# facebookresearch/NasRec

Measured on AMD Instinct MI355X. Metric: supernet samples/sec at batch 256 (Criteo-shape), 1/2/4/8 MI355X, higher is better.
Workload: dtype f32

## Files before the change

### nasrec_amd/csrc/worklist_body.h

```cpp
#pragma once
#include "attention_tok.h"
#include "gemm_rt.h"
#include "final_bodies.h"
#include "interact_bodies.h"
#include "dedup_bodies.h"

#define WL_LDS_BIG_FLOATS 9888
#define WL_LDS_FLOATS 7840
static_assert(MHA_TOK_BWD_LDS_FLOATS <= WL_LDS_BIG_FLOATS && MHA_TOK_FWD_LDS_FLOATS <= WL_LDS_FLOATS, "Transformer bodies fit the worklist launches");

#define WL_TK 64
#ifndef WL_AUX_RING2
#define WL_AUX_RING2 0
#endif
enum { WL_TOKS = 0, WL_T32x32 = 1, WL_T64x16 = 2, WL_T16x64 = 3 };

extern __shared__ __attribute__((aligned(16))) float wl_lds[];

template <typename T>
__device__ __forceinline__ const T& wl_ref(unsigned long long addr) {
  const unsigned lo = __builtin_amdgcn_readfirstlane((unsigned)addr), hi = __builtin_amdgcn_readfirstlane((unsigned)(addr >> 32));
  return *(const T*)(const __attribute__((address_space(4))) T*)(((unsigned long long)hi << 32) | lo);
}

template <bool KCA, bool KCB, int TBM, int TBN, bool AUX>
__device__ __forceinline__ void wl_gemm_cfg(unsigned long long blob, int vb_, int gx_, int gy_) {
  constexpr int RING = (AUX && !WL_AUX_RING2) ? 1 : 2;
  const nasrec_gemm_desc_t& g = wl_ref<nasrec_gemm_desc_t>(blob);
  const int vb = __builtin_amdgcn_readfirstlane(vb_), gx = __builtin_amdgcn_readfirstlane(gx_), gy = __builtin_amdgcn_readfirstlane(gy_);
  const int nprob = g.zmode ? g.nseg : 1;
  int Mmax = 0, Nmax = 0;
  for (int q = 0; q < nprob; ++q) {
    Mmax = max(Mmax, g.seg[q].M);
    Nmax = max(Nmax, g.seg[q].N);
  }
  const int bx = vb % gx, by = (vb / gx) % gy, bz = vb / (gx * gy);
  gemm_tile_rt<KCA, KCB, 256, WL_TK, TBM, TBN, AUX, RING>(g, Mmax, Nmax, bx, by, bz, wl_lds);
}

template <bool KCA, bool KCB, bool AUX>
__device__ __forceinline__ void wl_gemm_tile(int tile, unsigned long long off, int vb, int gx, int gy) {
  switch (tile) {
    case WL_T32x32: wl_gemm_cfg<KCA, KCB, 32, 32, AUX>(off, vb, gx, gy); break;
    case WL_T64x16: wl_gemm_cfg<KCA, KCB, 64, 16, AUX>(off, vb, gx, gy); break;
    default: wl_gemm_cfg<KCA, KCB, 16, 64, AUX>(off, vb, gx, gy); break;
  }
}

template <bool AUX>
__device__ __forceinline__ void wl_gemm_bind(int bind, int tile, unsigned long long off, int vb, int gx, int gy) {
  if (bind == 0) wl_gemm_tile<true, true, AUX>(tile, off, vb, gx, gy);
  else if (bind == 1) wl_gemm_tile<true, false, AUX>(tile, off, vb, gx, gy);
  else wl_gemm_tile<false, false, AUX>(tile, off, vb, gx, gy);
}

__device__ __forceinline__ void wl_warm_blob(unsigned long long addr, int bytes) {
  int sink, off;
  asm volatile(
      "s_mov_b32 %1, 0\n"
      "1:\n"
      "s_load_dword %0, %2, %1\n"
      "s_add_u32 %1, %1, 64\n"
      "s_cmp_lt_u32 %1, %3\n"
      "s_cbranch_scc1 1b\n"
      "s_waitcnt lgkmcnt(0)"
      : "=&s"(sink), "=&s"(off)
      : "s"(addr), "s"(bytes)
      : "scc", "memory");
}

#define WL_TOK_DEPTH 4
__device__ __forceinline__ void wl_token_fwd(unsigned long long blob, int vb_, int MT_) {
  const nasrec_gemm_desc_t& g = wl_ref<nasrec_gemm_desc_t>(blob);
  const int vb = __builtin_amdgcn_readfirstlane(vb_), MT = __builtin_amdgcn_readfirstlane(MT_);
  const int lane = threadIdx.x & 63, wave = __builtin_amdgcn_readfirstlane(threadIdx.x >> 6);
  const int e = lane & 15, fg = lane >> 4;
  wl_warm_blob(blob, (int)offsetof(nasrec_gemm_desc_t, seg) + g.nseg * (int)sizeof(nasrec_gemm_seg_t));
  const nasrec_gemm_seg_t& s0 = g.seg[0];
  const int M = s0.M, B = s0.N >> 4;
  const int unit = vb * 4 + wave;
  const int b = unit / MT, mt = unit - b * MT;
  if (b >= B) return;
  const int row = min(mt * 16 + e, M - 1);
  f32x4 acc = {0.f, 0.f, 0.f, 0.f};
  f32x4 fa[WL_TOK_DEPTH];
  float fb[WL_TOK_DEPTH][4];
  int lim[WL_TOK_DEPTH];
  int fq = 0, fk = 0;
  auto fetch = [&](int slot) {
    const bool in = fq < g.nseg;
    const nasrec_gemm_seg_t& sg = g.seg[in ? fq : 0];
    const bool live = in && sg.A != nullptr && sg.K > 0;
    const int K = live ? sg.K : 0, kk = fk + 4 * fg;
    lim[slot] = K - fk;
    const __amdgpu_buffer_rsrc_t ra =
        __builtin_amdgcn_make_buffer_rsrc(const_cast<float*>(sg.A), 0, live ? (int)(4 * ((long)(M - 1) * sg.lda + K)) : 0, 0x00020000);
    const __amdgpu_buffer_rsrc_t rb =
        __builtin_amdgcn_make_buffer_rsrc(const_cast<float*>(sg.B + (long)b * sg.ldb), 0, live ? 64 * K : 0, 0x00020000);
    fa[slot] = __builtin_bit_cast(f32x4, __builtin_amdgcn_raw_buffer_load_b128(ra, 4 * (row * sg.lda + kk), 0, 0));
#pragma unroll
    for (int j = 0; j < 4; ++j) fb[slot][j] = __builtin_bit_cast(float, __builtin_amdgcn_raw_buffer_load_b32(rb, 64 * (kk + j) + 4 * e, 0, 0));
    fk += 16;
    const bool next = fk >= K;
    fq = next ? fq + 1 : fq;
    fk = next ? 0 : fk;
  };
  auto multiply = [&](int slot) {
    const int l = lim[slot];
    if (l <= 0) return;
    f32x4 a = fa[slot];
    if (l < 16) {
#pragma unroll
      for (int j = 0; j < 4; ++j) a[j] = 4 * fg + j < l ? a[j] : 0.f;
    }
#pragma unroll
    for (int j = 0; j < 4; ++j) acc = __builtin_amdgcn_mfma_f32_16x16x4f32(a[j], fb[slot][j], acc, 0, 0, 0);
  };
  int steps = 0;
  for (int q = 0; q < g.nseg; ++q) steps += (g.seg[q].A && g.seg[q].K > 0) ? (g.seg[q].K + 15) >> 4 : 1;
#pragma unroll
  for (int r = 0; r < WL_TOK_DEPTH; ++r) fetch(r);
  for (int t = 0; t < steps; t += WL_TOK_DEPTH) {
#pragma unroll
    for (int r = 0; r < WL_TOK_DEPTH; ++r) {
      multiply(r);
      fetch(r);
    }
  }
  {
    const float v4[4] = {acc[0], acc[1], acc[2], acc[3]};
    if (mt * 16 + 4 * fg < M) epilogue_store_col4<NASREC_CM_TOKJ>(g, s0, mt * 16 + 4 * fg, b * 16 + e, M, v4);
  }
}

#define WL_DENSE_STEPS 8
__device__ __forceinline__ void wl_dense_small(unsigned long long blob, int vb_, int NT_, int MTNB_) {
  const nasrec_gemm_desc_t& g = wl_ref<nasrec_gemm_desc_t>(blob);
  const int vb = __builtin_amdgcn_readfirstlane(vb_), NT = __builtin_amdgcn_readfirstlane(NT_);
  const int MT = __builtin_amdgcn_readfirstlane(MTNB_) & 0xffff, NB = __builtin_amdgcn_readfirstlane(MTNB_) >> 16;
  const int lane = threadIdx.x & 63, wave = __builtin_amdgcn_readfirstlane(threadIdx.x >> 6);
  const int e = lane & 15, fg = lane >> 4;
  wl_warm_blob(blob, (int)offsetof(nasrec_gemm_desc_t, seg) + g.nseg * (int)sizeof(nasrec_gemm_seg_t));
  const nasrec_gemm_seg_t& s0 = g.seg[0];
  const int M = s0.M, N = s0.N;
  const int unit = vb * 4 + wave;
  if (unit >= MT * NT) return;
  const int mt = unit / NT, nt = unit - mt * NT;
  const int row = min(mt * 16 + e, M - 1), col = min(nt * 16 + e, N - 1);
  f32x4 fa[WL_DENSE_STEPS], fb[WL_DENSE_STEPS];
  int lim[WL_DENSE_STEPS];
  int fq = 0, fk = 0;
  f32x4 acc = {0.f, 0.f, 0.f, 0.f};
  for (int batch = 0; batch < NB; ++batch) {
#pragma unroll
  for (int slot = 0; slot < WL_DENSE_STEPS; ++slot) {
    const bool in = fq < g.nseg;
    const nasrec_gemm_seg_t& sg = g.seg[in ? fq : 0];
    const bool live = in && sg.A != nullptr && sg.K > 0;
    const int K = live ? sg.K : 0, kk = fk + 4 * fg;
    lim[slot] = K - fk;
    const __amdgpu_buffer_rsrc_t ra =
        __builtin_amdgcn_make_buffer_rsrc(const_cast<float*>(sg.A), 0, live ? (int)(4 * ((long)(M - 1) * sg.lda + K)) : 0, 0x00020000);
    const __amdgpu_buffer_rsrc_t rb =
        __builtin_amdgcn_make_buffer_rsrc(const_cast<float*>(sg.B), 0, live ? (int)(4 * ((long)(N - 1) * sg.ldb + K)) : 0, 0x00020000);
    fa[slot] = __builtin_bit_cast(f32x4, __builtin_amdgcn_raw_buffer_load_b128(ra, 4 * (row * sg.lda + kk), 0, 0));
    fb[slot] = __builtin_bit_cast(f32x4, __builtin_amdgcn_raw_buffer_load_b128(rb, 4 * (col * sg.ldb + kk), 0, 0));
    fk += 16;
    const bool next = fk >= K;
    fq = next ? fq + 1 : fq;
    fk = next ? 0 : fk;
  }
  if (batch == 0 && g.bias) {
    const float warm = g.bias[g.bias_on_rows ? row : col];
    asm volatile("" ::"v"(warm));
  }
#pragma unroll
  for (int slot = 0; slot < WL_DENSE_STEPS; ++slot) {
    const int l = lim[slot];
    if (l > 0) {
      f32x4 a = fa[slot], b = fb[slot];
      if (l < 16) {
#pragma unroll
        for (int j = 0; j < 4; ++j) {
          const bool in = 4 * fg + j < l;
          a[j] = in ? a[j] : 0.f;
          b[j] = in ? b[j] : 0.f;
        }
      }
#pragma unroll
      for (int j = 0; j < 4; ++j) acc = __builtin_amdgcn_mfma_f32_16x16x4f32(a[j], b[j], acc, 0, 0, 0);
    }
  }
  }
  {
    const float v4[4] = {acc[0], acc[1], acc[2], acc[3]};
    if (mt * 16 + 4 * fg < M && nt * 16 + e < N) epilogue_store_col4<NASREC_CM_PLAIN>(g, s0, mt * 16 + 4 * fg, nt * 16 + e, M, v4);
  }
}

__device__ __forceinline__ void wl_dense_small_dx(unsigned long long blob, int vb_, int TU_) {
  const nasrec_gemm_desc_t& g = wl_ref<nasrec_gemm_desc_t>(blob);
  const int vb = __builtin_amdgcn_readfirstlane(vb_), TU = __builtin_amdgcn_readfirstlane(TU_);
  const int lane = threadIdx.x & 63, wave = __builtin_amdgcn_readfirstlane(threadIdx.x >> 6);
  const int e = lane & 15, fg = lane >> 4;
  wl_warm_blob(blob, (int)offsetof(nasrec_gemm_desc_t, seg) + g.nseg * (int)sizeof(nasrec_gemm_seg_t));
  int t = vb * 4 + wave, q = 0;
  if (t >= TU) return;
  while (q < g.nseg - 1 && t >= ((g.seg[q].M + 15) >> 4) * ((g.seg[q].N + 15) >> 4)) t -= ((g.seg[q].M + 15) >> 4) * ((g.seg[q].N + 15) >> 4), ++q;
  const nasrec_gemm_seg_t& sg = g.seg[q];
  const int M = sg.M, N = sg.N, K = sg.K, NT = (N + 15) >> 4;
  const int mt = t / NT, nt = t - mt * NT;
  if (!sg.A || K <= 0) {
    if (!sg.accumulate) {
#pragma unroll
      for (int r = 0; r < 4; ++r) {
        const int i = mt * 16 + 4 * fg + r, j = nt * 16 + e;
        if (i < M && j < N) epilogue_store<NASREC_CM_PLAIN>(g, sg, i, j, 0.f);
      }
    }
    return;
  }
  const int row = min(mt * 16 + e, M - 1), col = min(nt * 16 + e, N - 1);
  const __amdgpu_buffer_rsrc_t ra = __builtin_amdgcn_make_buffer_rsrc(const_cast<float*>(sg.A), 0, (int)(4 * ((long)(M - 1) * sg.lda + K)), 0x00020000);
  const float* wp = sg.B + col;
  f32x4 fa[WL_DENSE_STEPS];
  float fb[WL_DENSE_STEPS][4];
#pragma unroll
  for (int s = 0; s < WL_DENSE_STEPS; ++s) {
    fa[s] = __builtin_bit_cast(f32x4, __builtin_amdgcn_raw_buffer_load_b128(ra, 4 * (row * sg.lda + 16 * s + 4 * fg), 0, 0));
#pragma unroll
    for (int j = 0; j < 4; ++j) fb[s][j] = wp[(long)min(16 * s + 4 * fg + j, K - 1) * sg.ldb];
  }
  if (sg.Aaux) {
    const __amdgpu_buffer_rsrc_t rx = __builtin_amdgcn_make_buffer_rsrc(const_cast<float*>(sg.Aaux), 0, (int)(4 * ((long)(M - 1) * sg.lda + K)), 0x00020000);
    f32x4 fx[WL_DENSE_STEPS];
#pragma unroll
    for (int s = 0; s < WL_DENSE_STEPS; ++s) fx[s] = __builtin_bit_cast(f32x4, __builtin_amdgcn_raw_buffer_load_b128(rx, 4 * (row * sg.lda + 16 * s + 4 * fg), 0, 0));
#pragma unroll
    for (int s = 0; s < WL_DENSE_STEPS; ++s)
#pragma unroll
      for (int j = 0; j < 4; ++j) fa[s][j] = fx[s][j] > 0.f ? fa[s][j] : 0.f;
  }
  f32x4 acc = {0.f, 0.f, 0.f, 0.f};
#pragma unroll
  for (int s = 0; s < WL_DENSE_STEPS; ++s) {
    if (16 * s < K) {
#pragma unroll
      for (int j = 0; j < 4; ++j) {
        const bool in = 16 * s + 4 * fg + j < K;
        acc = __builtin_amdgcn_mfma_f32_16x16x4f32(in ? fa[s][j] : 0.f, in ? fb[s][j] : 0.f, acc, 0, 0, 0);
      }
    }
  }
  {
    const float v4[4] = {acc[0], acc[1], acc[2], acc[3]};
    if (mt * 16 + 4 * fg < M && nt * 16 + e < N) epilogue_store_col4<NASREC_CM_PLAIN>(g, sg, mt * 16 + 4 * fg, nt * 16 + e, M, v4);
  }
}

#define WL_TOKDX_STEPS 4
#define WL_TOK_MAX_WG (1 << 20)
__device__ __forceinline__ void wl_token_dx_unit(const nasrec_gemm_desc_t& g, int unit, int TU, int e, int fg);
__device__ __forceinline__ void wl_token_dx(unsigned long long blob, int vb_, int TU_) {
  const nasrec_gemm_desc_t& g = wl_ref<nasrec_gemm_desc_t>(blob);
  const int vb = __builtin_amdgcn_readfirstlane(vb_), TU = __builtin_amdgcn_readfirstlane(TU_);
  const int lane = threadIdx.x & 63, wave = __builtin_amdgcn_readfirstlane(threadIdx.x >> 6);
  wl_warm_blob(blob, (int)offsetof(nasrec_gemm_desc_t, seg) + g.nseg * (int)sizeof(nasrec_gemm_seg_t));
  const int total = (g.seg[0].N >> 4) * TU, stride = 4 * min((total + 3) >> 2, WL_TOK_MAX_WG);
  for (int unit = vb * 4 + wave; unit < total; unit += stride) wl_token_dx_unit(g, unit, TU, lane & 15, lane >> 4);
}
__device__ __forceinline__ void wl_token_dx_unit(const nasrec_gemm_desc_t& g, int unit, int TU, int e, int fg) {
  const int b = unit / TU;
  int t = unit - b * TU, q = 0;
  while (q < g.nseg && t >= ((g.seg[q].M + 15) >> 4)) t -= (g.seg[q].M + 15) >> 4, ++q;
  const nasrec_gemm_seg_t& sg = g.seg[q];
  const int M = sg.M, K = sg.K;
  if (!sg.A || K <= 0) {
    if (!sg.accumulate) {
#pragma unroll
      for (int r = 0; r < 4; ++r) {
        const int i = t * 16 + 4 * fg + r;
        if (i < M) epilogue_store<NASREC_CM_TOKJ>(g, sg, i, b * 16 + e, 0.f);
      }
    }
    return;
  }
  const int row = min(t * 16 + e, M - 1);
  const float* wp = sg.A + row;
  const float* yb = sg.B + (long)b * sg.ldb + e;
  float fa[WL_TOKDX_STEPS][4], fb[WL_TOKDX_STEPS][4];
#pragma unroll
  for (int s = 0; s < WL_TOKDX_STEPS; ++s)
#pragma unroll
    for (int j = 0; j < 4; ++j) {
      const int k = min(16 * s + 4 * fg + j, K - 1);
      fa[s][j] = wp[(long)k * sg.lda];
      fb[s][j] = yb[k * 16];
    }
  if (sg.Baux) {
    const float* xb = sg.Baux + (long)b * sg.ldb + e;
    float fx[WL_TOKDX_STEPS][4];
#pragma unroll
    for (int s = 0; s < WL_TOKDX_STEPS; ++s)
#pragma unroll
      for (int j = 0; j < 4; ++j) fx[s][j] = xb[min(16 * s + 4 * fg + j, K - 1) * 16];
#pragma unroll
    for (int s = 0; s < WL_TOKDX_STEPS; ++s)
#pragma unroll
      for (int j = 0; j < 4; ++j) fb[s][j] = fx[s][j] > 0.f ? fb[s][j] : 0.f;
  }
  f32x4 acc = {0.f, 0.f, 0.f, 0.f};
#pragma unroll
  for (int s = 0; s < WL_TOKDX_STEPS; ++s) {
    if (16 * s < K) {
#pragma unroll
      for (int j = 0; j < 4; ++j) {
        const bool in = 16 * s + 4 * fg + j < K;
        acc = __builtin_amdgcn_mfma_f32_16x16x4f32(in ? fa[s][j] : 0.f, in ? fb[s][j] : 0.f, acc, 0, 0, 0);
      }
    }
  }
  {
    const float v4[4] = {acc[0], acc[1], acc[2], acc[3]};
    if (t * 16 + 4 * fg < M) epilogue_store_col4<NASREC_CM_TOKJ>(g, sg, t * 16 + 4 * fg, b * 16 + e, M, v4);
  }
}

__device__ __forceinline__ void wl_gemm_second_pass(unsigned long long blob, int vb_, int per_) {
  const nasrec_gemm_desc_t& g = wl_ref<nasrec_gemm_desc_t>(blob);
  const int vb = __builtin_amdgcn_readfirstlane(vb_), per = __builtin_amdgcn_readfirstlane(per_);
  const int nprob = g.zmode ? g.nseg : 1;
  int Mmax = 0, Nmax = 0;
  for (int q = 0; q < nprob; ++q) {
    Mmax = max(Mmax, g.seg[q].M);
    Nmax = max(Nmax, g.seg[q].N);
  }
  const int z = vb / per;
  const long e = (long)(vb - z * per) * 256 + threadIdx.x;
  if (g.cmode == NASREC_CM_PLAIN)
    splitk_second_pass<NASREC_CM_PLAIN>(g, Mmax, Nmax, z, e);
  else
    splitk_second_pass<NASREC_CM_TOKJ>(g, Mmax, Nmax, z, e);
}

__device__ __forceinline__ void wl_mha_fwd(unsigned long long blob, int vb) {
  mha_fwd_tok(wl_ref<nasrec_mha_desc_t>(blob), __builtin_amdgcn_readfirstlane(vb), wl_lds);
}

#define WL_PACKED_NONE 0xffffffffu
#define WL_HEAD_BYTES 48
template <bool BIG>
__device__ __forceinline__ void wl_run(unsigned f01, unsigned f23, unsigned f45, unsigned f67, unsigned f89, unsigned fab, unsigned m01, unsigned m23,
                                       unsigned m45, unsigned m67, unsigned m89, unsigned mab, const unsigned long long base) {
  const nasrec_worklist_desc_t& wl = wl_ref<nasrec_worklist_desc_t>(base);
  float* lds = wl_lds;
  const int bid = blockIdx.x, tid = threadIdx.x, wave = tid >> 6, lane = tid & 63;
  int k = 0, it_first = 0, it_kind, it_part, it_off;
  if (f01 != WL_PACKED_NONE) {
    const unsigned f[6] = {f01, f23, f45, f67, f89, fab}, m[6] = {m01, m23, m45, m67, m89, mab};
    unsigned meta = m01 & 0xffffu;
#pragma unroll
    for (int q = 1; q < NASREC_WL_MAX_ITEMS; ++q) {
      const unsigned fq = (f[q >> 1] >> (16 * (q & 1))) & 0xffffu, mq = (m[q >> 1] >> (16 * (q & 1))) & 0xffffu;
      if ((unsigned)bid >= fq) {
        k = q;
        it_first = (int)fq;
        meta = mq;
      }
    }
    it_kind = meta & 63;
    it_part = (meta >> 6) & 3;
    it_off = (int)(meta >> 8) * 16;
  } else {
#pragma unroll 1
    while (k + 1 < wl.n && bid >= wl.item[k + 1].first) ++k;
    it_first = wl.item[k].first;
    it_kind = wl.item[k].kind;
    it_part = wl.item[k].part;
    it_off = wl.item[k].off;
  }
  const nasrec_wl_item_t& it = wl.item[k];
  const int vb = bid - it_first;
  const unsigned long long blob = base + offsetof(nasrec_worklist_desc_t, blob) + it_off;
  switch (it_kind) {
    case NASREC_OP_GEMM: {
      if (it_part == 2) {
        wl_gemm_second_pass(blob, vb, it.geom[0]);
        break;
      }
      const int cfg = it.geom[2];
      if ((cfg & 3) == WL_TOKS && ((cfg >> 2) & 3) == 3 && it.geom[1] == 0) wl_dense_small_dx(blob, vb, it.geom[0]);
      else if ((cfg & 3) == WL_TOKS && ((cfg >> 2) & 3) == 3) wl_dense_small(blob, vb, it.geom[0], it.geom[1]);
      else if ((cfg & 3) == WL_TOKS && ((cfg >> 2) & 3) == 1) wl_token_fwd(blob, vb, it.geom[0]);
      else if ((cfg & 3) == WL_TOKS) wl_token_dx(blob, vb, it.geom[0]);
      else if ((cfg >> 4) & 1) wl_gemm_bind<true>((cfg >> 2) & 3, cfg & 3, blob, vb, it.geom[0], it.geom[1]);
      else wl_gemm_bind<false>((cfg >> 2) & 3, cfg & 3, blob, vb, it.geom[0], it.geom[1]);
      break;
    }
    case NASREC_OP_MHA_FWD:
      wl_mha_fwd(blob, vb);
      break;
    case NASREC_OP_MHA_BWD:
      if (BIG) mha_bwd_tok(wl_ref<nasrec_mha_desc_t>(blob), __builtin_amdgcn_readfirstlane(vb), wl_lds);
      break;
    case NASREC_OP_FM_FWD: {
      const nasrec_fm_desc_t& d = wl_ref<nasrec_fm_desc_t>(blob);
      const int b = vb * 4 + wave;
      if (b < d.B) fm_fwd_sample(d, b, lane);
      break;
    }
    case NASREC_OP_FM_BWD: {
      const nasrec_fm_desc_t& d = wl_ref<nasrec_fm_desc_t>(blob);
      const int b = vb * 4 + wave;
      if (b < d.B) fm_bwd_sample(d, b, lane);
      break;
    }
    case NASREC_OP_DOT_TRI_FWD: {
      const nasrec_dot_tri_desc_t& d = wl_ref<nasrec_dot_tri_desc_t>(blob);
      const int b = vb * 4 + wave;
      if (b < d.B) dot_tri_fwd_sample(d, b, lane, lds + wave * (d.k1 * TRI_LD));
      break;
    }
    case NASREC_OP_DOT_TRI_BWD: {
      const nasrec_dot_tri_desc_t& d = wl_ref<nasrec_dot_tri_desc_t>(blob);
      const int b = vb * 4 + wave;
      const int P4 = (d.k1 * (d.k1 - 1) / 2 + 3) & ~3;
      if (b < d.B) dot_tri_bwd_sample(d, b, lane, lds + wave * (d.k1 * TRI_LD), lds + 4 * (d.k1 * TRI_LD) + wave * P4);
      break;
    }
    case NASREC_OP_COPY_SEGS: {
      const nasrec_copy_segs_desc_t& d = wl_ref<nasrec_copy_segs_desc_t>(blob);
      const int W = it.geom[0];
      const long t = (long)vb * 256 + tid;
      if (t < (long)d.B * W) copy_segs_element(d, (int)(t / W), (int)(t % W));
      break;
    }
    case NASREC_OP_GATE_BWD:
      gate_bwd_element(wl_ref<nasrec_gate_bwd_desc_t>(blob), (long)vb * 256 + tid);
      break;
    case NASREC_OP_REDUCE_ROWS:
      reduce_rows_block(wl_ref<nasrec_wl_reduce_t>(blob), vb, tid, lds);
      break;
    case NASREC_OP_DEDUP_IDS: {
      const nasrec_dedup_ids_desc_t& d = wl_ref<nasrec_dedup_ids_desc_t>(blob);
      dedup_ids_small_body(d, d.idx, d.B, d.Fs, __builtin_amdgcn_readfirstlane(vb), reinterpret_cast<int*>(lds), reinterpret_cast<int*>(lds) + 256);
      break;
    }
    case NASREC_OP_FINAL_FWD:
      final_fwd_block(wl_ref<nasrec_final_desc_t>(blob), __builtin_amdgcn_readfirstlane(vb), lds);
      break;
    case NASREC_OP_FINAL_FUSED:
      final_fused_block(wl_ref<nasrec_final_desc_t>(blob), __builtin_amdgcn_readfirstlane(vb), lds);
      break;
    case NASREC_OP_FINAL_BWD:
      final_bwd_block(wl_ref<nasrec_final_desc_t>(blob), it.geom[0], it.geom[1], it.geom[2], __builtin_amdgcn_readfirstlane(vb), lds);
      break;
    default:
      break;
  }
}

template <bool BIG>
__global__ __launch_bounds__(256, 4) void worklist_kernel(unsigned f01, unsigned f23, unsigned f45, unsigned f67, unsigned f89, unsigned fab,
                                                                    unsigned m01, unsigned m23, unsigned m45, unsigned m67, unsigned m89, unsigned mab,
                                                                    const nasrec_worklist_desc_t wl) {
  wl_run<BIG>(f01, f23, f45, f67, f89, fab, m01, m23, m45, m67, m89, mab, (unsigned long long)__builtin_amdgcn_kernarg_segment_ptr() + WL_HEAD_BYTES);
}
template <bool BIG>
__global__ __launch_bounds__(256, 4) void worklist_dev_kernel(unsigned f01, unsigned f23, unsigned f45, unsigned f67, unsigned f89, unsigned fab,
                                                                        unsigned m01, unsigned m23, unsigned m45, unsigned m67, unsigned m89, unsigned mab,
                                                                        const nasrec_worklist_desc_t* wl) {
  wl_run<BIG>(f01, f23, f45, f67, f89, fab, m01, m23, m45, m67, m89, mab, (unsigned long long)wl);
}
```

Baseline: 1.162 million.

## Issue all token-GEMM loads up front for short K and pair X loads

For token forward GEMMs with few K-steps (up to 13), a templated path issues every A and X load before any MFMA, so all memory latency overlaps at once instead of passing through a depth-4 ring. X is read as two 64-bit loads per lane and redistributed with a DPP lane swap, replacing four scalar 32-bit loads. A bias value is also touched early to warm its cache line. The cost is higher register pressure from the fully unrolled C-slot buffers and three template instantiations, which could lower occupancy or cause spills. Longer K still uses the old pipelined loop.

After: 1.171 million (median of 6 runs). Within noise of the previous version (+0.8%).

```diff
diff --git a/nasrec_amd/csrc/worklist_body.h b/nasrec_amd/csrc/worklist_body.h
--- a/nasrec_amd/csrc/worklist_body.h
+++ b/nasrec_amd/csrc/worklist_body.h
@@ -70,6 +70,62 @@
 }
 
 #define WL_TOK_DEPTH 4
+#define WL_TOK_INFLIGHT 13
+template <int C>
+__device__ __forceinline__ f32x4 wl_token_inflight(const nasrec_gemm_desc_t& g, int M, int b, int row, int e, int fg) {
+  f32x4 acc = {0.f, 0.f, 0.f, 0.f};
+  f32x4 wa[C];
+  f32x2 xa[C][2];
+  int lim[C];
+  const int odd = e & 1;
+  const int xoff = 64 * (4 * fg + odd) + 4 * (e & 14);
+  int q = 0, k0 = 0, K = 0, lda = 0;
+  __amdgpu_buffer_rsrc_t ra, rb;
+  auto enter = [&]() {
+    const float *A = nullptr, *X = nullptr;
+    K = 0;
+    if (q < g.nseg) {
+      const nasrec_gemm_seg_t& sg = g.seg[q];
+      A = sg.A, X = sg.B + (long)b * sg.ldb, lda = sg.lda;
+      K = (A != nullptr && sg.K > 0) ? sg.K : 0;
+    }
+    ra = __builtin_amdgcn_make_buffer_rsrc(const_cast<float*>(A), 0, K > 0 ? (int)(4 * ((long)(M - 1) * lda + K)) : 0, 0x00020000);
+    rb = __builtin_amdgcn_make_buffer_rsrc(const_cast<float*>(X), 0, 64 * K, 0x00020000);
+  };
+  const __amdgpu_buffer_rsrc_t rbias = __builtin_amdgcn_make_buffer_rsrc(const_cast<float*>(g.bias), 0, (g.bias && g.bias_on_rows) ? 4 * M : 0, 0x00020000);
+  const int warm = __builtin_amdgcn_raw_buffer_load_b32(rbias, 4 * row, 0, 0);
+  enter();
+#pragma unroll
+  for (int s = 0; s < C; ++s) {
+    lim[s] = K - k0;
+    wa[s] = __builtin_bit_cast(f32x4, __builtin_amdgcn_raw_buffer_load_b128(ra, 4 * (row * lda + k0 + 4 * fg), 0, 0));
+#pragma unroll
+    for (int t = 0; t < 2; ++t) xa[s][t] = __builtin_bit_cast(f32x2, __builtin_amdgcn_raw_buffer_load_b64(rb, 64 * k0 + xoff + 128 * t, 0, 0));
+    k0 += 16;
+    if (k0 >= K) {
+      ++q, k0 = 0;
+      enter();
+    }
+  }
+#pragma unroll
+  for (int s = 0; s < C; ++s) {
+    const int l = lim[s];
+    if (l > 0) {
+      f32x4 a = wa[s];
+      if (l < 16) {
+#pragma unroll
+        for (int j = 0; j < 4; ++j) a[j] = 4 * fg + j < l ? a[j] : 0.f;
+      }
+      const float r0 = dpp_mov<0xb1>(odd ? xa[s][0][0] : xa[s][0][1]), r1 = dpp_mov<0xb1>(odd ? xa[s][1][0] : xa[s][1][1]);
+      const float x[4] = {odd ? r0 : xa[s][0][0], odd ? xa[s][0][1] : r0, odd ? r1 : xa[s][1][0], odd ? xa[s][1][1] : r1};
+#pragma unroll
+      for (int j = 0; j < 4; ++j) acc = __builtin_amdgcn_mfma_f32_16x16x4f32(a[j], x[j], acc, 0, 0, 0);
+    }
+  }
+  asm volatile("" ::"v"(warm));
+  return acc;
+}
+
 __device__ __forceinline__ void wl_token_fwd(unsigned long long blob, int vb_, int MT_) {
   const nasrec_gemm_desc_t& g = wl_ref<nasrec_gemm_desc_t>(blob);
   const int vb = __builtin_amdgcn_readfirstlane(vb_), MT = __builtin_amdgcn_readfirstlane(MT_);
@@ -82,49 +138,57 @@
   const int b = unit / MT, mt = unit - b * MT;
   if (b >= B) return;
   const int row = min(mt * 16 + e, M - 1);
-  f32x4 acc = {0.f, 0.f, 0.f, 0.f};
-  f32x4 fa[WL_TOK_DEPTH];
-  float fb[WL_TOK_DEPTH][4];
-  int lim[WL_TOK_DEPTH];
-  int fq = 0, fk = 0;
-  auto fetch = [&](int slot) {
-    const bool in = fq < g.nseg;
-    const nasrec_gemm_seg_t& sg = g.seg[in ? fq : 0];
-    const bool live = in && sg.A != nullptr && sg.K > 0;
-    const int K = live ? sg.K : 0, kk = fk + 4 * fg;
-    lim[slot] = K - fk;
-    const __amdgpu_buffer_rsrc_t ra =
-        __builtin_amdgcn_make_buffer_rsrc(const_cast<float*>(sg.A), 0, live ? (int)(4 * ((long)(M - 1) * sg.lda + K)) : 0, 0x00020000);
-    const __amdgpu_buffer_rsrc_t rb =
-        __builtin_amdgcn_make_buffer_rsrc(const_cast<float*>(sg.B + (long)b * sg.ldb), 0, live ? 64 * K : 0, 0x00020000);
-    fa[slot] = __builtin_bit_cast(f32x4, __builtin_amdgcn_raw_buffer_load_b128(ra, 4 * (row * sg.lda + kk), 0, 0));
-#pragma unroll
-    for (int j = 0; j < 4; ++j) fb[slot][j] = __builtin_bit_cast(float, __builtin_amdgcn_raw_buffer_load_b32(rb, 64 * (kk + j) + 4 * e, 0, 0));
-    fk += 16;
-    const bool next = fk >= K;
-    fq = next ? fq + 1 : fq;
-    fk = next ? 0 : fk;
-  };
-  auto multiply = [&](int slot) {
-    const int l = lim[slot];
-    if (l <= 0) return;
-    f32x4 a = fa[slot];
-    if (l < 16) {
-#pragma unroll
-      for (int j = 0; j < 4; ++j) a[j] = 4 * fg + j < l ? a[j] : 0.f;
-    }
-#pragma unroll
-    for (int j = 0; j < 4; ++j) acc = __builtin_amdgcn_mfma_f32_16x16x4f32(a[j], fb[slot][j], acc, 0, 0, 0);
-  };
   int steps = 0;
   for (int q = 0; q < g.nseg; ++q) steps += (g.seg[q].A && g.seg[q].K > 0) ? (g.seg[q].K + 15) >> 4 : 1;
-#pragma unroll
-  for (int r = 0; r < WL_TOK_DEPTH; ++r) fetch(r);
-  for (int t = 0; t < steps; t += WL_TOK_DEPTH) {
-#pragma unroll
-    for (int r = 0; r < WL_TOK_DEPTH; ++r) {
-      multiply(r);
-      fetch(r);
+  f32x4 acc = {0.f, 0.f, 0.f, 0.f};
+  if (steps <= 4) {
+    acc = wl_token_inflight<4>(g, M, b, row, e, fg);
+  } else if (steps <= 8) {
+    acc = wl_token_inflight<8>(g, M, b, row, e, fg);
+  } else if (steps <= WL_TOK_INFLIGHT) {
+    acc = wl_token_inflight<WL_TOK_INFLIGHT>(g, M, b, row, e, fg);
+  } else {
+    f32x4 fa[WL_TOK_DEPTH];
+    float fb[WL_TOK_DEPTH][4];
+    int lim[WL_TOK_DEPTH];
+    int fq = 0, fk = 0;
+    auto fetch = [&](int slot) {
+      const bool in = fq < g.nseg;
+      const nasrec_gemm_seg_t& sg = g.seg[in ? fq : 0];
+      const bool live = in && sg.A != nullptr && sg.K > 0;
+      const int K = live ? sg.K : 0, kk = fk + 4 * fg;
+      lim[slot] = K - fk;
+      const __amdgpu_buffer_rsrc_t ra =
+          __builtin_amdgcn_make_buffer_rsrc(const_cast<float*>(sg.A), 0, live ? (int)(4 * ((long)(M - 1) * sg.lda + K)) : 0, 0x00020000);
+      const __amdgpu_buffer_rsrc_t rb =
+          __builtin_amdgcn_make_buffer_rsrc(const_cast<float*>(sg.B + (long)b * sg.ldb), 0, live ? 64 * K : 0, 0x00020000);
+      fa[slot] = __builtin_bit_cast(f32x4, __builtin_amdgcn_raw_buffer_load_b128(ra, 4 * (row * sg.lda + kk), 0, 0));
+#pragma unroll
+      for (int j = 0; j < 4; ++j) fb[slot][j] = __builtin_bit_cast(float, __builtin_amdgcn_raw_buffer_load_b32(rb, 64 * (kk + j) + 4 * e, 0, 0));
+      fk += 16;
+      const bool next = fk >= K;
+      fq = next ? fq + 1 : fq;
+      fk = next ? 0 : fk;
+    };
+    auto multiply = [&](int slot) {
+      const int l = lim[slot];
+      if (l <= 0) return;
+      f32x4 a = fa[slot];
+      if (l < 16) {
+#pragma unroll
+        for (int j = 0; j < 4; ++j) a[j] = 4 * fg + j < l ? a[j] : 0.f;
+      }
+#pragma unroll
+      for (int j = 0; j < 4; ++j) acc = __builtin_amdgcn_mfma_f32_16x16x4f32(a[j], fb[slot][j], acc, 0, 0, 0);
+    };
+#pragma unroll
+    for (int r = 0; r < WL_TOK_DEPTH; ++r) fetch(r);
+    for (int t = 0; t < steps; t += WL_TOK_DEPTH) {
+#pragma unroll
+      for (int r = 0; r < WL_TOK_DEPTH; ++r) {
+        multiply(r);
+        fetch(r);
+      }
     }
   }
   {
```
